# wubinzzu/NeuRec

Measured on NVIDIA H100. Metric: triplets/sec, higher is better.
Workload: dtype f32

## Files before the change

### neurec_b200/csrc/epoch.cuh

```cuda
#pragma once
#include "common.cuh"
#include "philox.cuh"

namespace nrc {

constexpr int kFeistelRounds = 8;

struct Feistel {
    uint32_t key[kFeistelRounds];
    uint64_t n;
    int32_t bits_l;
    int32_t bits_r;
    int32_t shuffle;
};

__host__ __device__ __forceinline__ uint32_t feistel_mix(uint32_t r, uint32_t key) {
    const uint32_t v = r ^ key;
    const uint64_t prod = (uint64_t)0xD2511F53u * v;
    uint32_t f = (uint32_t)(prod >> 32) ^ (uint32_t)prod;
    f = (f ^ (f >> 15)) * 0x9E3779B1u;
    return f ^ (f >> 13);
}

__host__ __device__ __forceinline__ uint64_t feistel_once(const Feistel& F, uint64_t x) {
    int bl = F.bits_l, br = F.bits_r;
    uint32_t L = (uint32_t)(x >> br), R = (uint32_t)(x & ((1ull << br) - 1ull));
#pragma unroll
    for (int r = 0; r < kFeistelRounds; ++r) {
        const uint32_t nr = L ^ (feistel_mix(R, F.key[r]) & (uint32_t)((1ull << bl) - 1ull));
        L = R; R = nr;
        const int t = bl; bl = br; br = t;
    }
    return ((uint64_t)L << br) | R;
}

__host__ __device__ __forceinline__ int64_t feistel_perm(const Feistel& F, int64_t p) {
    if (!F.shuffle) return p;
    uint64_t x = (uint64_t)p;
    do { x = feistel_once(F, x); } while (x >= F.n);
    return (int64_t)x;
}

struct EpochSpec {
    const int64_t* tptr;
    const int32_t* tidx;
    const int32_t* users;
    const int32_t* pos;
    int64_t n_pos;
    int64_t n_samples;
    int32_t neg_num;
    int32_t num_items;
    int32_t pairwise;
    uint64_t seed, stream_id;
    Feistel perm;
};

__device__ __forceinline__ void epoch_sample(const EpochSpec& E, int64_t p, int k, int32_t& u, int32_t& item,
                                             int32_t& third) {
    const int64_t idx = feistel_perm(E.perm, p);
    if (E.pairwise) {
        u = __ldg(E.users + idx);
        item = __ldg(E.pos + idx);
        const int64_t beg = __ldg(E.tptr + u);
        third = philox_draw_excluding((uint64_t)(idx * E.neg_num + k), E.seed, E.stream_id, E.num_items,
                                      E.tidx + beg, __ldg(E.tptr + u + 1) - beg);
    } else if (idx < E.n_pos) {
        u = __ldg(E.users + idx);
        item = __ldg(E.pos + idx);
        third = __float_as_int(1.0f);
    } else {
        const int64_t t = idx - E.n_pos;
        const int64_t kk = t / E.n_pos, q = t - kk * E.n_pos;
        u = __ldg(E.users + q);
        const int64_t beg = __ldg(E.tptr + u);
        item = philox_draw_excluding((uint64_t)(q * E.neg_num + kk), E.seed, E.stream_id, E.num_items,
                                     E.tidx + beg, __ldg(E.tptr + u + 1) - beg);
        third = __float_as_int(0.0f);
    }
}

int feistel_init(Feistel& F, int64_t n, int shuffle, uint64_t seed, uint64_t epoch);
int epoch_spec_init(EpochSpec& E, const int64_t* tptr, const int32_t* tidx, const int32_t* users, const int32_t* pos,
                    int64_t n_pos, int32_t neg_num, int32_t num_items, int32_t pairwise, int32_t shuffle,
                    uint64_t seed, uint64_t stream_id);

__device__ __forceinline__ void grid_barrier(unsigned int* counter, unsigned int& target) {
    __syncthreads();
    if (threadIdx.x == 0) {
        target += gridDim.x;
        unsigned int seen;
        asm volatile("red.release.gpu.global.add.u32 [%0], 1;" ::"l"(counter) : "memory");
        do {
            asm volatile("ld.acquire.gpu.global.u32 %0, [%1];" : "=r"(seen) : "l"(counter) : "memory");
        } while (seen < target);
    }
    __syncthreads();
}

}
```

### neurec_b200/csrc/train_mf.cu

```cuda
#include <stdlib.h>

#include "common.cuh"
#include "epoch.cuh"
#include "learner.cuh"
#include "mf.cuh"
#include "optim.cuh"

namespace nrc {

template <bool PAIRWISE>
__global__ void __launch_bounds__(256)
mf_grad_kernel(const float* __restrict__ U, const float* __restrict__ V, int D, const int32_t* __restrict__ users,
               const int32_t* __restrict__ items, const int32_t* __restrict__ third, int64_t batch, int loss_kind,
               float reg, float* __restrict__ gU, float* __restrict__ gV, int32_t* __restrict__ tU,
               int32_t* __restrict__ tV, int32_t stamp, float* __restrict__ loss) {
    const int lane = threadIdx.x & 31;
    const int wib = threadIdx.x >> 5;
    const int wpb = blockDim.x >> 5;
    const float inv_b = 1.0f / (float)batch;
    float loss_acc = 0.0f;
    for (int64_t b = (int64_t)blockIdx.x * wpb + wib; b < batch; b += (int64_t)gridDim.x * wpb)
        loss_acc += mf_sample_grad<PAIRWISE, 0, false>(U, V, gU, gV, tU, tV, D, reg, loss_kind, lane, users[b], items[b],
                                                       third[b], inv_b, stamp);
    if (lane == 0 && loss) atomicAdd(loss, loss_acc);
}

struct RowShards {
    float* base[8];
    int32_t rows_per_shard;
    int32_t self;
    int32_t vec_remote;
    int32_t force_remote;
    float* hot;
    float* hot_delta;
    int32_t n_hot;
    template <bool SHARDED>
    __device__ __forceinline__ float* row(int32_t id, int D, bool& remote, float*& upd) const {
        if (id < n_hot) {
            remote = false;
            upd = hot_delta + (size_t)id * D;
            return hot + (size_t)id * D;
        }
        float* p = row<SHARDED>(id, D, remote);
        upd = p;
        return p;
    }
    template <bool SHARDED>
    __device__ __forceinline__ float* row(int32_t id, int D, bool& remote) const {
        if constexpr (!SHARDED) {
            remote = force_remote != 0;
            return base[0] + (size_t)id * D;
        } else {
            const int32_t owner = id / rows_per_shard;
            remote = owner != self || force_remote;
            float* b = base[0];
#pragma unroll
            for (int r = 1; r < 8; ++r) b = (owner == r) ? base[r] : b;
            return b + (size_t)(id - owner * rows_per_shard) * D;
        }
    }
};

template <int VEC>
__device__ __forceinline__ void red_row(float* p, const float (&d)[VEC], bool remote) {
    if (remote) {
#pragma unroll
        for (int t = 0; t < VEC; ++t) atomicAdd(p + t, d[t]);
        return;
    }
    red_vec<VEC>(p, d);
}

template <int VEC, bool SHARDED>
__global__ void __launch_bounds__(256)
mf_bpr_sgd_fused_kernel(const RowShards U, const RowShards V, const int32_t* __restrict__ users,
                        const int32_t* __restrict__ pos, const int32_t* __restrict__ neg, int64_t batch,
                        float lr, float reg, float* __restrict__ loss) {
    constexpr int D = 32 * VEC;
    const int lane = threadIdx.x & 31;
    const int64_t wpb = blockDim.x >> 5;
    float loss_acc = 0.0f;
    for (int64_t b = (int64_t)blockIdx.x * wpb + (threadIdx.x >> 5); b < batch; b += (int64_t)gridDim.x * wpb) {
        bool ru, ri, rj;
        float* pu = U.row<SHARDED>(users[b], D, ru) + lane * VEC;
        float* qi = V.row<SHARDED>(pos[b], D, ri) + lane * VEC;
        float* qj = V.row<SHARDED>(neg[b], D, rj) + lane * VEC;
        float a[VEC], bi[VEC], bj[VEC];
        ld_vec<VEC>(pu, a); ld_vec<VEC>(qi, bi); ld_vec<VEC>(qj, bj);
        float di = 0.f, dj = 0.f, sq = 0.f;
#pragma unroll
        for (int t = 0; t < VEC; ++t) {
            di = fmaf(a[t], bi[t], di);
            dj = fmaf(a[t], bj[t], dj);
            sq += a[t] * a[t] + bi[t] * bi[t] + bj[t] * bj[t];
        }
        di = warp_sum(di); dj = warp_sum(dj);
        const float x = di - dj;
        float l = neg_log_sigmoid(x);
        if (reg != 0.0f) l += reg * 0.5f * warp_sum(sq);
        loss_acc += l;
        const float g = neg_log_sigmoid_grad(x);
        float du[VEC], dvi[VEC], dvj[VEC];
#pragma unroll
        for (int t = 0; t < VEC; ++t) {
            du[t] = -lr * (g * (bi[t] - bj[t]) + reg * a[t]);
            dvi[t] = -lr * (g * a[t] + reg * bi[t]);
            dvj[t] = -lr * (-g * a[t] + reg * bj[t]);
        }
        red_row<VEC>(pu, du, ru && U.vec_remote == 0);
        red_row<VEC>(qi, dvi, ri && V.vec_remote == 0);
        red_row<VEC>(qj, dvj, rj && V.vec_remote == 0);
    }
    if (lane == 0 && loss) atomicAdd(loss, loss_acc);
}

static int peer_red_mode() {
    static int vec = -1;
    if (vec < 0) { const char* e = getenv("NRC_PEER_VEC_RED"); vec = e ? atoi(e) : 1; }
    return vec;
}

static int launch_bpr_sgd(const RowShards& SU, const RowShards& SV, int dim, const int32_t* users,
                          const int32_t* pos, const int32_t* neg, int64_t batch, float lr, float reg, float* loss,
                          cudaStream_t st) {
    int64_t blocks = (batch + 7) / 8;
    const int64_t cap = (int64_t)sm_count() * 8;
    if (blocks > cap) blocks = cap;
    const unsigned gb = (unsigned)blocks;
#define NRC_LAUNCH_SGD(VEC, SH) \
    mf_bpr_sgd_fused_kernel<VEC, SH><<<gb, 256, 0, st>>>(SU, SV, users, pos, neg, batch, lr, reg, loss)
    const bool sharded = SU.rows_per_shard != 0;
    if (dim == 128) { if (sharded) NRC_LAUNCH_SGD(4, true); else NRC_LAUNCH_SGD(4, false); }
    else if (dim == 64) { if (sharded) NRC_LAUNCH_SGD(2, true); else NRC_LAUNCH_SGD(2, false); }
    else { if (sharded) NRC_LAUNCH_SGD(1, true); else NRC_LAUNCH_SGD(1, false); }
#undef NRC_LAUNCH_SGD
    NRC_CUDA_CHECK(cudaGetLastError());
    return NRC_OK;
}


template <int VEC>
constexpr int kSgdTierRows = 8192 / (32 * VEC);
template <int VEC>
constexpr size_t kSgdTierBytes = (size_t)2 * kSgdTierRows<VEC> * 32 * VEC * sizeof(float);

template <int VEC, bool SHARDED>
__device__ __forceinline__ void load_item(const RowShards& V, int32_t id, int nt, const float* s_val, int lane,
                                          float (&v)[VEC]) {
    if (id < nt) {
        ld_vec<VEC>(s_val + id * (32 * VEC) + lane * VEC, v);
    } else {
        bool remote;
        float* upd;
        ld_vec<VEC>(V.row<SHARDED>(id, 32 * VEC, remote, upd) + lane * VEC, v);
    }
}

template <int VEC, bool SHARDED>
__device__ __forceinline__ void update_item(const RowShards& V, int32_t id, int nt, float* s_dlt, int lane,
                                            const float (&d)[VEC]) {
    if (id < nt) {
#pragma unroll
        for (int t = 0; t < VEC; ++t) atomicAdd(s_dlt + id * (32 * VEC) + t * 32 + lane, d[t]);
    } else {
        bool remote;
        float* upd;
        V.row<SHARDED>(id, 32 * VEC, remote, upd);
        red_row<VEC>(upd + lane * VEC, d, remote && V.vec_remote == 0);
    }
}

constexpr int kStreamThreads = 768;

template <int VEC, bool SHARDED>
__global__ void __launch_bounds__(kStreamThreads, 1)
mf_bpr_sgd_stream_kernel(float* __restrict__ U_local, const RowShards V, const EpochSpec E, int64_t first,
                         int64_t count, float lr, float reg, float* __restrict__ loss) {
    constexpr int D = 32 * VEC, CH = kStreamThreads, T = kSgdTierRows<VEC>;
    constexpr int TPW = 2;
    __shared__ int32_t s_u[CH], s_i[CH], s_j[CH];
    extern __shared__ __align__(16) float s_tier[];
    float* const s_val = s_tier;
    float* const s_dlt = s_tier + T * D;
    const int lane = threadIdx.x & 31, warp = threadIdx.x >> 5;
    const int nt = V.n_hot < T ? V.n_hot : T;
    for (int e = threadIdx.x; e < nt * D / 4; e += blockDim.x) {
        reinterpret_cast<float4*>(s_val)[e] = reinterpret_cast<const float4*>(V.hot)[e];
        reinterpret_cast<float4*>(s_dlt)[e] = make_float4(0.f, 0.f, 0.f, 0.f);
    }
    const int64_t lo = count * blockIdx.x / gridDim.x, hi = count * (blockIdx.x + 1) / gridDim.x;
    float loss_acc = 0.0f;
    for (int64_t c0 = lo; c0 < hi; c0 += CH) {
        const int n = (hi - c0 < CH) ? (int)(hi - c0) : CH;
        if ((int)threadIdx.x < n) {
            int32_t u, i, j;
            epoch_sample(E, first + c0 + threadIdx.x, 0, u, i, j);
            s_u[threadIdx.x] = u; s_i[threadIdx.x] = i; s_j[threadIdx.x] = j;
        }
        __syncthreads();
        for (int t0 = warp * TPW; t0 < n; t0 += (kStreamThreads / 32) * TPW) {
            float a[TPW][VEC], b[TPW][VEC], c[TPW][VEC];
#pragma unroll
            for (int k = 0; k < TPW; ++k) {
                const int t = (t0 + k < n) ? t0 + k : t0;
                ld_vec<VEC>(U_local + (size_t)s_u[t] * D + lane * VEC, a[k]);
                load_item<VEC, SHARDED>(V, s_i[t], nt, s_val, lane, b[k]);
                load_item<VEC, SHARDED>(V, s_j[t], nt, s_val, lane, c[k]);
            }
            float di[TPW], dj[TPW], sq[TPW];
#pragma unroll
            for (int k = 0; k < TPW; ++k) {
                di[k] = 0.f; dj[k] = 0.f; sq[k] = 0.f;
#pragma unroll
                for (int t = 0; t < VEC; ++t) {
                    di[k] = fmaf(a[k][t], b[k][t], di[k]); dj[k] = fmaf(a[k][t], c[k][t], dj[k]);
                    sq[k] += a[k][t] * a[k][t] + b[k][t] * b[k][t] + c[k][t] * c[k][t];
                }
                di[k] = warp_sum(di[k]); dj[k] = warp_sum(dj[k]);
            }
#pragma unroll
            for (int k = 0; k < TPW; ++k) {
                if (t0 + k >= n) break;
                const int t = t0 + k;
                const float x = di[k] - dj[k];
                float l = neg_log_sigmoid(x);
                if (reg != 0.0f) l += reg * 0.5f * warp_sum(sq[k]);
                loss_acc += l;
                const float g = neg_log_sigmoid_grad(x);
                float du[VEC], dvi[VEC], dvj[VEC];
#pragma unroll
                for (int q = 0; q < VEC; ++q) {
                    du[q] = -lr * (g * (b[k][q] - c[k][q]) + reg * a[k][q]);
                    dvi[q] = -lr * (g * a[k][q] + reg * b[k][q]);
                    dvj[q] = -lr * (-g * a[k][q] + reg * c[k][q]);
                }
                red_row<VEC>(U_local + (size_t)s_u[t] * D + lane * VEC, du, false);
                update_item<VEC, SHARDED>(V, s_i[t], nt, s_dlt, lane, dvi);
                update_item<VEC, SHARDED>(V, s_j[t], nt, s_dlt, lane, dvj);
            }
        }
        __syncthreads();
    }
    __syncthreads();
    for (int e = threadIdx.x; e < nt * 32; e += blockDim.x) {
        const int r = e >> 5, l = e & 31;
        float d[VEC];
        bool any = false;
#pragma unroll
        for (int t = 0; t < VEC; ++t) { d[t] = s_dlt[r * D + t * 32 + l]; any |= d[t] != 0.0f; }
        if (any) red_row<VEC>(V.hot_delta + (size_t)r * D + l * VEC, d, false);
    }
    if (lane == 0 && loss) atomicAdd(loss, loss_acc);
}

template <int VEC, bool SH>
static int launch_stream(float* U_local, const RowShards& SV, const EpochSpec& E, int64_t first, int64_t count, float lr,
                         float reg, float* loss, cudaStream_t st) {
    constexpr size_t smem = kSgdTierBytes<VEC>;
    static int64_t grid_cap = 0;
    if (!grid_cap) {
        NRC_CUDA_CHECK(cudaFuncSetAttribute(mf_bpr_sgd_stream_kernel<VEC, SH>, cudaFuncAttributeMaxDynamicSharedMemorySize,
                                            (int)smem));
        int per_sm = 0;
        NRC_CUDA_CHECK(cudaOccupancyMaxActiveBlocksPerMultiprocessor(&per_sm, mf_bpr_sgd_stream_kernel<VEC, SH>, kStreamThreads, smem));
        NRC_REQUIRE(per_sm > 0, NRC_E_CUDA, "mf_bpr_sgd_stream_kernel does not fit on an SM");
        grid_cap = (int64_t)per_sm * sm_count();
    }
    int64_t blocks = (count + kStreamThreads - 1) / kStreamThreads;
    if (blocks > grid_cap) blocks = grid_cap;
    mf_bpr_sgd_stream_kernel<VEC, SH><<<(unsigned)blocks, kStreamThreads, smem, st>>>(U_local, SV, E, first, count, lr, reg, loss);
    NRC_CUDA_CHECK(cudaGetLastError());
    return NRC_OK;
}

static int launch_bpr_sgd_stream(float* U_local, const RowShards& SV, int dim, const EpochSpec& E, int64_t first,
                                 int64_t count, float lr, float reg, float* loss, cudaStream_t st) {
    const bool sharded = SV.rows_per_shard != 0;
#define NRC_STREAM(VEC) (sharded ? launch_stream<VEC, true>(U_local, SV, E, first, count, lr, reg, loss, st) \
                                 : launch_stream<VEC, false>(U_local, SV, E, first, count, lr, reg, loss, st))
    if (dim == 128) return NRC_STREAM(4);
    if (dim == 64) return NRC_STREAM(2);
    return NRC_STREAM(1);
#undef NRC_STREAM
}

template <int VEC>
__device__ __forceinline__ void lazy_adam_row(float* var, float* m, float* v, const float (&x)[VEC], float (&mm)[VEC],
                                              float (&vv)[VEC], const float (&g)[VEC], float lr_t, float b1, float b2,
                                              float eps) {
    float out[VEC];
#pragma unroll
    for (int t = 0; t < VEC; ++t) {
        mm[t] = b1 * mm[t] + (1.0f - b1) * g[t];
        vv[t] = b2 * vv[t] + (1.0f - b2) * g[t] * g[t];
        out[t] = x[t] - lr_t * mm[t] / (sqrtf(vv[t]) + eps);
    }
    st_vec<VEC>(m, mm); st_vec<VEC>(v, vv); st_vec<VEC>(var, out);
}

template <int VEC>
__global__ void __launch_bounds__(256, 3)
mf_bpr_lazy_adam_stream_kernel(float* __restrict__ U, float* __restrict__ mU, float* __restrict__ vU, float* __restrict__ V,
                               float* __restrict__ mV, float* __restrict__ vV, const EpochSpec E, int64_t first, int64_t count,
                               float lr_t, float b1, float b2, float eps, float reg, float* __restrict__ loss) {
    constexpr int D = 32 * VEC;
    constexpr int CH = 256;
    __shared__ int32_t s_u[CH], s_i[CH], s_j[CH];
    const int lane = threadIdx.x & 31, warp = threadIdx.x >> 5;
    float loss_acc = 0.0f;
    for (int64_t c0 = (int64_t)blockIdx.x * CH; c0 < count; c0 += (int64_t)gridDim.x * CH) {
        const int n = (count - c0 < CH) ? (int)(count - c0) : CH;
        if ((int)threadIdx.x < n) {
            int32_t u, i, j;
            epoch_sample(E, first + c0 + threadIdx.x, 0, u, i, j);
            s_u[threadIdx.x] = u; s_i[threadIdx.x] = i; s_j[threadIdx.x] = j;
        }
        __syncthreads();
        for (int t = warp; t < n; t += 8) {
            const size_t ou = (size_t)s_u[t] * D + lane * VEC, oi = (size_t)s_i[t] * D + lane * VEC,
                         oj = (size_t)s_j[t] * D + lane * VEC;
            float a[VEC], bi[VEC], bj[VEC], mu[VEC], vu[VEC], mi[VEC], vi[VEC], mj[VEC], vj[VEC];
            ld_vec<VEC>(U + ou, a); ld_vec<VEC>(V + oi, bi); ld_vec<VEC>(V + oj, bj);
            ld_vec<VEC>(mU + ou, mu); ld_vec<VEC>(vU + ou, vu);
            ld_vec<VEC>(mV + oi, mi); ld_vec<VEC>(vV + oi, vi);
            ld_vec<VEC>(mV + oj, mj); ld_vec<VEC>(vV + oj, vj);
            float di = 0.f, dj = 0.f, sq = 0.f;
#pragma unroll
            for (int c = 0; c < VEC; ++c) {
                di = fmaf(a[c], bi[c], di); dj = fmaf(a[c], bj[c], dj);
                sq += a[c] * a[c] + bi[c] * bi[c] + bj[c] * bj[c];
            }
            di = warp_sum(di); dj = warp_sum(dj);
            const float x = di - dj;
            float l = neg_log_sigmoid(x);
            if (reg != 0.0f) l += reg * 0.5f * warp_sum(sq);
            loss_acc += l;
            const float g = neg_log_sigmoid_grad(x);
            float gu[VEC], gi[VEC], gj[VEC];
#pragma unroll
            for (int c = 0; c < VEC; ++c) {
                gu[c] = g * (bi[c] - bj[c]) + reg * a[c];
                gi[c] = g * a[c] + reg * bi[c];
                gj[c] = -g * a[c] + reg * bj[c];
            }
            lazy_adam_row<VEC>(U + ou, mU + ou, vU + ou, a, mu, vu, gu, lr_t, b1, b2, eps);
            lazy_adam_row<VEC>(V + oi, mV + oi, vV + oi, bi, mi, vi, gi, lr_t, b1, b2, eps);
            lazy_adam_row<VEC>(V + oj, mV + oj, vV + oj, bj, mj, vj, gj, lr_t, b1, b2, eps);
        }
        __syncthreads();
    }
    if (lane == 0 && loss) atomicAdd(loss, loss_acc);
}

static int grad_grid(int64_t batch) {
    const int wpb = 8;
    int64_t blocks = (batch + wpb - 1) / wpb;
    const int64_t cap = (int64_t)sm_count() * 8;
    if (blocks > cap) blocks = cap;
    if (blocks < 1) blocks = 1;
    return (int)blocks;
}

}

using namespace nrc;

extern "C" int nrc_mf_pairwise_grad(const float* user_table, const float* item_table, int32_t dim,
                                    const int32_t* users, const int32_t* pos_items,
                                    const int32_t* neg_items, int64_t batch, int32_t loss_kind,
                                    float reg, float* grad_user, float* grad_item,
                                    int32_t* touched_user, int32_t* touched_item, int32_t stamp,
                                    float* loss, void* stream) {
    NRC_REQUIRE(loss_kind == NRC_LOSS_BPR || loss_kind == NRC_LOSS_HINGE ||
                    loss_kind == NRC_LOSS_SQUARE,
                NRC_E_VALUE, "please choose a suitable loss function");
    NRC_REQUIRE(dim > 0 && batch >= 0, NRC_E_VALUE, "dim must be positive, batch >= 0");
    if (batch == 0) return NRC_OK;
    mf_grad_kernel<true><<<grad_grid(batch), 256, 0, as_stream(stream)>>>(
        user_table, item_table, dim, users, pos_items, neg_items, batch, loss_kind, reg, grad_user,
        grad_item, touched_user, touched_item, stamp, loss);
    NRC_CUDA_CHECK(cudaGetLastError());
    return NRC_OK;
}

extern "C" int nrc_mf_pointwise_grad(const float* user_table, const float* item_table, int32_t dim,
                                     const int32_t* users, const int32_t* items,
                                     const float* labels, int64_t batch, int32_t loss_kind,
                                     float reg, float* grad_user, float* grad_item,
                                     int32_t* touched_user, int32_t* touched_item, int32_t stamp,
                                     float* loss, void* stream) {
    NRC_REQUIRE(loss_kind == NRC_LOSS_CROSS_ENTROPY || loss_kind == NRC_LOSS_SQUARE, NRC_E_VALUE,
                "please choose a suitable loss function");
    NRC_REQUIRE(dim > 0 && batch >= 0, NRC_E_VALUE, "dim must be positive, batch >= 0");
    if (batch == 0) return NRC_OK;
    mf_grad_kernel<false><<<grad_grid(batch), 256, 0, as_stream(stream)>>>(
        user_table, item_table, dim, users, items, reinterpret_cast<const int32_t*>(labels), batch, loss_kind, reg,
        grad_user, grad_item, touched_user, touched_item, stamp, loss);
    NRC_CUDA_CHECK(cudaGetLastError());
    return NRC_OK;
}

extern "C" int nrc_mf_bpr_sgd_fused(float* user_table, float* item_table, int32_t dim,
                                    const int32_t* users, const int32_t* pos_items,
                                    const int32_t* neg_items, int64_t batch, float lr, float reg,
                                    float* loss, void* stream) {
    NRC_REQUIRE(dim == 32 || dim == 64 || dim == 128, NRC_E_LIMIT,
                "the fused single-pass step supports dim 32, 64 or 128 (got %d)", dim);
    NRC_REQUIRE(batch >= 0, NRC_E_VALUE, "batch must be >= 0");
    if (batch == 0) return NRC_OK;
    RowShards SU{}, SV{};
    SU.base[0] = user_table; SV.base[0] = item_table;
    return launch_bpr_sgd(SU, SV, dim, users, pos_items, neg_items, batch, lr, reg, loss, as_stream(stream));
}

extern "C" int nrc_mf_bpr_sgd_sharded(float* const* user_shards, float* const* item_shards, int32_t world,
                                      int32_t self_rank, int64_t users_per_shard, int64_t items_per_shard, int32_t dim,
                                      const int32_t* users, const int32_t* pos_items, const int32_t* neg_items,
                                      int64_t batch, float lr, float reg, float* loss, void* stream) {
    NRC_REQUIRE(world >= 1 && world <= 8, NRC_E_LIMIT, "world %d outside [1, 8]", world);
    NRC_REQUIRE(self_rank >= 0 && self_rank < world, NRC_E_VALUE, "self_rank %d outside [0, %d)", self_rank, world);
    NRC_REQUIRE(user_shards != nullptr && item_shards != nullptr, NRC_E_VALUE, "shard pointer arrays are NULL");
    NRC_REQUIRE(users_per_shard > 0 && items_per_shard > 0 && users_per_shard < (1ll << 31) &&
                    items_per_shard < (1ll << 31) && users_per_shard * world < (1ll << 31) &&
                    items_per_shard * world < (1ll << 31),
                NRC_E_LIMIT, "global row ids must fit int32");
    NRC_REQUIRE(dim == 32 || dim == 64 || dim == 128, NRC_E_LIMIT, "fused SGD supports dim 32, 64, 128 (got %d)", dim);
    if (batch <= 0) return NRC_OK;
    RowShards SU{}, SV{};
    for (int r = 0; r < world; ++r) {
        NRC_REQUIRE(user_shards[r] != nullptr && item_shards[r] != nullptr, NRC_E_VALUE, "shard %d is NULL", r);
        SU.base[r] = user_shards[r];
        SV.base[r] = item_shards[r];
    }
    SU.rows_per_shard = (int32_t)users_per_shard;
    SV.rows_per_shard = (int32_t)items_per_shard;
    SU.self = SV.self = self_rank;
    SU.vec_remote = SV.vec_remote = peer_red_mode();
    return launch_bpr_sgd(SU, SV, dim, users, pos_items, neg_items, batch, lr, reg, loss, as_stream(stream));
}

extern "C" int nrc_mf_bpr_sgd_epoch_hot(float* user_table, float* const* item_shards, int32_t world, int32_t self_rank,
                                    int64_t items_per_shard, int32_t dim, const int64_t* train_indptr,
                                    const int32_t* train_indices, const int32_t* pos_users, const int32_t* pos_items,
                                    int64_t n_pos, int32_t num_items, int32_t shuffle, uint64_t seed, uint64_t epoch,
                                    int64_t first, int64_t count, float lr, float reg, float* loss, float* hot, float* hot_delta,
                                    int32_t n_hot, void* stream) {
    NRC_REQUIRE(world >= 1 && world <= 8, NRC_E_LIMIT, "world %d outside [1, 8]", world);
    NRC_REQUIRE(self_rank >= 0 && self_rank < world, NRC_E_VALUE, "self_rank %d outside [0, %d)", self_rank, world);
    NRC_REQUIRE(user_table != nullptr && item_shards != nullptr, NRC_E_VALUE, "table pointers are NULL");
    NRC_REQUIRE(dim == 32 || dim == 64 || dim == 128, NRC_E_LIMIT, "fused SGD supports dim 32, 64, 128 (got %d)", dim);
    NRC_REQUIRE(world == 1 || (items_per_shard > 0 && items_per_shard * world < (1ll << 31) &&
                               items_per_shard * world >= num_items),
                NRC_E_VALUE, "items_per_shard %lld x world %d must cover num_items %d and fit int32",
                (long long)items_per_shard, world, num_items);
    EpochSpec E;
    int rc = epoch_spec_init(E, train_indptr, train_indices, pos_users, pos_items, n_pos, 1, num_items, 1, shuffle, seed,
                             epoch);
    if (rc) return rc;
    NRC_REQUIRE(first >= 0 && count >= 0 && first + count <= n_pos, NRC_E_VALUE,
                "[first, first + count) = [%lld, %lld) outside the epoch's %lld triplets", (long long)first,
                (long long)(first + count), (long long)n_pos);
    if (count == 0) return NRC_OK;
    RowShards SV{};
    for (int r = 0; r < world; ++r) {
        NRC_REQUIRE(item_shards[r] != nullptr, NRC_E_VALUE, "item shard %d is NULL", r);
        SV.base[r] = item_shards[r];
    }
    SV.rows_per_shard = world > 1 ? (int32_t)items_per_shard : 0;
    SV.self = self_rank;
    NRC_REQUIRE(n_hot >= 0 && n_hot <= num_items && (n_hot == 0 || (hot != nullptr && hot_delta != nullptr)), NRC_E_VALUE,
                "n_hot %d needs 0 <= n_hot <= num_items and the replica / delta buffers", n_hot);
    SV.hot = hot; SV.hot_delta = hot_delta; SV.n_hot = n_hot;
    {
        static int vec = -1, force = -1;
        if (vec < 0) vec = peer_red_mode();
        if (force < 0) { const char* e = getenv("NRC_FORCE_REMOTE_PATH"); force = e ? atoi(e) : 0; }
        SV.vec_remote = vec;
        SV.force_remote = force;
    }
    return launch_bpr_sgd_stream(user_table, SV, dim, E, first, count, lr, reg, loss, as_stream(stream));
}

extern "C" int nrc_mf_bpr_sgd_epoch(float* user_table, float* const* item_shards, int32_t world, int32_t self_rank,
                                    int64_t items_per_shard, int32_t dim, const int64_t* train_indptr,
                                    const int32_t* train_indices, const int32_t* pos_users, const int32_t* pos_items,
                                    int64_t n_pos, int32_t num_items, int32_t shuffle, uint64_t seed, uint64_t epoch,
                                    int64_t first, int64_t count, float lr, float reg, float* loss, void* stream) {
    return nrc_mf_bpr_sgd_epoch_hot(user_table, item_shards, world, self_rank, items_per_shard, dim, train_indptr,
                                    train_indices, pos_users, pos_items, n_pos, num_items, shuffle, seed, epoch, first,
                                    count, lr, reg, loss, nullptr, nullptr, 0, stream);
}

namespace nrc {
__global__ void __launch_bounds__(256) hot_apply_kernel(float4* __restrict__ hot, float4* __restrict__ delta, int64_t n4) {
    for (int64_t e = (int64_t)blockIdx.x * blockDim.x + threadIdx.x; e < n4; e += (int64_t)gridDim.x * blockDim.x) {
        float4 h = hot[e];
        const float4 d = delta[e];
        h.x += d.x; h.y += d.y; h.z += d.z; h.w += d.w;
        hot[e] = h;
        delta[e] = make_float4(0.f, 0.f, 0.f, 0.f);
    }
}
}

extern "C" int nrc_mf_hot_apply(float* hot, float* hot_delta, int64_t n_floats, void* stream) {
    NRC_REQUIRE(n_floats >= 0 && (n_floats & 3) == 0, NRC_E_VALUE, "n_floats %lld must be a multiple of 4", (long long)n_floats);
    if (n_floats == 0) return NRC_OK;
    NRC_REQUIRE(hot && hot_delta, NRC_E_VALUE, "replica / delta pointers are NULL");
    int64_t blocks = (n_floats / 4 + 255) / 256;
    const int64_t cap = (int64_t)sm_count() * 8;
    if (blocks > cap) blocks = cap;
    hot_apply_kernel<<<(unsigned)blocks, 256, 0, as_stream(stream)>>>(reinterpret_cast<float4*>(hot),
                                                                      reinterpret_cast<float4*>(hot_delta), n_floats / 4);
    NRC_CUDA_CHECK(cudaGetLastError());
    return NRC_OK;
}

extern "C" int nrc_mf_bpr_lazy_adam_epoch(float* user_table, float* user_m, float* user_v, float* item_table, float* item_m,
                                          float* item_v, int32_t dim, const int64_t* train_indptr,
                                          const int32_t* train_indices, const int32_t* pos_users, const int32_t* pos_items,
                                          int64_t n_pos, int32_t num_items, int32_t shuffle, uint64_t seed, uint64_t epoch,
                                          int64_t first, int64_t count, float lr_t, float beta1, float beta2, float eps,
                                          float reg, float* loss, void* stream) {
    NRC_REQUIRE(dim == 32 || dim == 64 || dim == 128, NRC_E_LIMIT, "lazy Adam supports dim 32, 64, 128 (got %d)", dim);
    NRC_REQUIRE(user_table && user_m && user_v && item_table && item_m && item_v, NRC_E_VALUE, "table / slot pointers are NULL");
    EpochSpec E;
    int rc = epoch_spec_init(E, train_indptr, train_indices, pos_users, pos_items, n_pos, 1, num_items, 1, shuffle, seed,
                             epoch);
    if (rc) return rc;
    NRC_REQUIRE(first >= 0 && count >= 0 && first + count <= n_pos, NRC_E_VALUE,
                "[first, first + count) = [%lld, %lld) outside the epoch's %lld triplets", (long long)first,
                (long long)(first + count), (long long)n_pos);
    if (count == 0) return NRC_OK;
    int64_t blocks = (count + 255) / 256;
    const int64_t cap = (int64_t)sm_count() * 8;
    if (blocks > cap) blocks = cap;
    cudaStream_t st = as_stream(stream);
#define NRC_LAZY(VEC) mf_bpr_lazy_adam_stream_kernel<VEC><<<(unsigned)blocks, 256, 0, st>>>( \
        user_table, user_m, user_v, item_table, item_m, item_v, E, first, count, lr_t, beta1, beta2, eps, reg, loss)
    if (dim == 128) NRC_LAZY(4); else if (dim == 64) NRC_LAZY(2); else NRC_LAZY(1);
#undef NRC_LAZY
    NRC_CUDA_CHECK(cudaGetLastError());
    return NRC_OK;
}

extern "C" int nrc_enable_peer_access(int32_t peer_device) {
    int cur = 0;
    NRC_CUDA_CHECK(cudaGetDevice(&cur));
    if (cur == peer_device) return NRC_OK;
    int can = 0;
    NRC_CUDA_CHECK(cudaDeviceCanAccessPeer(&can, cur, peer_device));
    NRC_REQUIRE(can, NRC_E_CUDA, "device %d cannot access device %d", cur, peer_device);
    const cudaError_t e = cudaDeviceEnablePeerAccess(peer_device, 0);
    if (e == cudaErrorPeerAccessAlreadyEnabled) { cudaGetLastError(); return NRC_OK; }
    NRC_CUDA_CHECK(e);
    return NRC_OK;
}

extern "C" int nrc_opt_apply_rows(int32_t opt_kind, float* var, float* grad, float* slot0,
                                  float* slot1, const int32_t* touched, int32_t stamp, int64_t rows,
                                  int32_t dim, const float* hyper_host, void* stream) {
    OptLaunch L;
    int rc = opt_launch_init(L, opt_kind, hyper_host);
    if (rc) return rc;
    rc = opt_launch_add(L, var, grad, slot0, slot1, touched, rows, dim, 0);
    if (rc) return rc;
    return opt_launch_run(L, stamp, as_stream(stream));
}

extern "C" int nrc_opt_apply_multi(int32_t opt_kind, int32_t n_vars, float* const* var,
                                   float* const* grad, float* const* slot0, float* const* slot1,
                                   const int32_t* const* touched, const int64_t* rows,
                                   const int32_t* dims, const int32_t* dense_var, int32_t stamp,
                                   const float* hyper_host, void* stream) {
    OptLaunch L;
    int rc = opt_launch_init(L, opt_kind, hyper_host);
    if (rc) return rc;
    for (int i = 0; i < n_vars; ++i) {
        rc = opt_launch_add(L, var[i], grad[i], slot0 ? slot0[i] : nullptr,
                            slot1 ? slot1[i] : nullptr, touched ? touched[i] : nullptr, rows[i],
                            dims[i], dense_var ? dense_var[i] : 0);
        if (rc) return rc;
    }
    return opt_launch_run(L, stamp, as_stream(stream));
}

extern "C" int nrc_mf_train_epoch(float* user_table, float* item_table, int32_t num_users,
                                  int32_t num_items, int32_t dim, const int32_t* users,
                                  const int32_t* items, const void* third, int64_t n,
                                  int32_t batch_size, int32_t pairwise, int32_t loss_kind, float reg,
                                  int32_t opt_kind, const float* lr_t_host, const float* hyper_host,
                                  float* grad_user, float* grad_item, int32_t* touched_user,
                                  int32_t* touched_item, float* slot0_user, float* slot1_user,
                                  float* slot0_item, float* slot1_item, int32_t first_stamp,
                                  float* step_loss, void* stream) {
    NRC_REQUIRE(batch_size > 0, NRC_E_VALUE, "batch_size should be a positive integeral value");
    NRC_REQUIRE(n >= 0 && dim > 0, NRC_E_VALUE, "n >= 0 and dim > 0 required");
    cudaStream_t st = as_stream(stream);
    const int64_t steps = (n + batch_size - 1) / batch_size;
    if (steps == 0) return NRC_OK;
    NRC_CUDA_CHECK(cudaMemsetAsync(step_loss, 0, (size_t)steps * sizeof(float), st));
    float hyper[4] = {hyper_host[0], hyper_host[1], hyper_host[2], hyper_host[3]};
    for (int64_t s = 0; s < steps; ++s) {
        const int64_t off = s * batch_size;
        const int64_t bs = (n - off < batch_size) ? (n - off) : batch_size;
        const int32_t stamp = first_stamp + (int32_t)s;
        int rc;
        if (pairwise)
            rc = nrc_mf_pairwise_grad(user_table, item_table, dim, users + off, items + off,
                                      reinterpret_cast<const int32_t*>(third) + off, bs, loss_kind,
                                      reg, grad_user, grad_item, touched_user, touched_item, stamp,
                                      step_loss + s, stream);
        else
            rc = nrc_mf_pointwise_grad(user_table, item_table, dim, users + off, items + off,
                                       reinterpret_cast<const float*>(third) + off, bs, loss_kind,
                                       reg, grad_user, grad_item, touched_user, touched_item, stamp,
                                       step_loss + s, stream);
        if (rc) return rc;
        if (opt_kind == NRC_OPT_ADAM) hyper[0] = lr_t_host[s];
        OptLaunch L;
        rc = opt_launch_init(L, opt_kind, hyper);
        if (rc) return rc;
        opt_launch_add(L, user_table, grad_user, slot0_user, slot1_user, touched_user, num_users, dim, 0);
        opt_launch_add(L, item_table, grad_item, slot0_item, slot1_item, touched_item, num_items, dim, 0);
        rc = opt_launch_run(L, stamp, st);
        if (rc) return rc;
    }
    return NRC_OK;
}

extern "C" int nrc_mf_train_step_host(float* user_table, float* item_table, int32_t num_users,
                                      int32_t num_items, int32_t dim, const int32_t* users_host,
                                      const int32_t* items_host, const void* third_host,
                                      int64_t batch, int32_t pairwise, int32_t loss_kind, float reg,
                                      int32_t opt_kind, const float* hyper_host, float* grad_user,
                                      float* grad_item, int32_t* touched_user,
                                      int32_t* touched_item, float* slot0_user, float* slot1_user,
                                      float* slot0_item, float* slot1_item, int32_t stamp,
                                      void* staging, float* loss_host, void* stream) {
    NRC_REQUIRE(batch > 0 && dim > 0, NRC_E_VALUE, "batch and dim must be positive");
    cudaStream_t st = as_stream(stream);
    int32_t* d_users = reinterpret_cast<int32_t*>(staging);
    int32_t* d_items = d_users + batch;
    int32_t* d_third = d_items + batch;
    float* d_loss = reinterpret_cast<float*>(d_third + batch);
    const size_t nb = (size_t)batch * sizeof(int32_t);
    NRC_CUDA_CHECK(cudaMemcpyAsync(d_users, users_host, nb, cudaMemcpyHostToDevice, st));
    NRC_CUDA_CHECK(cudaMemcpyAsync(d_items, items_host, nb, cudaMemcpyHostToDevice, st));
    NRC_CUDA_CHECK(cudaMemcpyAsync(d_third, third_host, nb, cudaMemcpyHostToDevice, st));
    NRC_CUDA_CHECK(cudaMemsetAsync(d_loss, 0, sizeof(float), st));
    int rc;
    if (pairwise)
        rc = nrc_mf_pairwise_grad(user_table, item_table, dim, d_users, d_items, d_third, batch,
                                  loss_kind, reg, grad_user, grad_item, touched_user, touched_item,
                                  stamp, d_loss, stream);
    else
        rc = nrc_mf_pointwise_grad(user_table, item_table, dim, d_users, d_items,
                                   reinterpret_cast<const float*>(d_third), batch, loss_kind, reg,
                                   grad_user, grad_item, touched_user, touched_item, stamp, d_loss,
                                   stream);
    if (rc) return rc;
    OptLaunch L;
    rc = opt_launch_init(L, opt_kind, hyper_host);
    if (rc) return rc;
    opt_launch_add(L, user_table, grad_user, slot0_user, slot1_user, touched_user, num_users, dim, 0);
    opt_launch_add(L, item_table, grad_item, slot0_item, slot1_item, touched_item, num_items, dim, 0);
    rc = opt_launch_run(L, stamp, st);
    if (rc) return rc;
    NRC_CUDA_CHECK(cudaMemcpyAsync(loss_host, d_loss, sizeof(float), cudaMemcpyDeviceToHost, st));
    NRC_CUDA_CHECK(cudaStreamSynchronize(st));
    return NRC_OK;
}
```

### profiles/step_rows.py

```python
import argparse
import json
import os
import sys

import numpy as np

ROOT = os.path.dirname(os.path.dirname(os.path.abspath(__file__)))
sys.path.insert(0, ROOT)


def main():
    import bench
    import oracle
    ap = argparse.ArgumentParser()
    ap.add_argument("--step", type=int, default=0)
    args = ap.parse_args()
    cfg = bench.ShardedCfg
    ptr, idx = bench.synth_shard_csr(cfg, 0, 1, device="cpu")
    users = np.repeat(np.arange(len(ptr) - 1, dtype=np.int32), np.diff(ptr))
    wu, wi, wj = oracle.epoch_build(ptr, idx, users, idx, 1, cfg.items_per_gpu, True, True, bench.SEED, 0)
    lo = args.step * cfg.batch
    u, i, j = wu[lo:lo + cfg.batch], wi[lo:lo + cfg.batch], wj[lo:lo + cfg.batch, 0]
    n_hot = bench.n_hot_of(cfg, 1)
    cu = np.bincount(u, minlength=cfg.users_per_gpu)
    items = np.concatenate([i, j])
    ci = np.bincount(items[items >= n_hot], minlength=cfg.items_per_gpu)
    once_u = int((cu[u] == 1).sum())
    cold_i, cold_j = i[i >= n_hot], j[j >= n_hot]
    once_i, once_j = int((ci[cold_i] == 1).sum()), int((ci[cold_j] == 1).sum())
    total = len(u) + len(cold_i) + len(cold_j)
    print(json.dumps({
        "step": args.step, "triplets": len(u), "n_hot": n_hot,
        "user_updates": len(u), "user_touched_once": once_u / len(u),
        "negative_updates_outside_head": len(cold_j), "negatives_in_head": float((j < n_hot).mean()),
        "negative_touched_once": once_j / len(cold_j),
        "positive_updates_outside_head": len(cold_i), "positive_touched_once": once_i / len(cold_i),
        "positives_in_head": int((i < n_hot).sum()), "positives_in_shared_memory_tier": int((i < 64).sum()),
        "in_place_updates": total, "touched_once": once_u + once_i + once_j,
        "touched_once_share": (once_u + once_i + once_j) / total}))


if __name__ == "__main__":
    main()
```

Measured before the change: 837.9 million.

## Replace atomic user-row updates with plain stores for users touched once per chunk

For each sampled triplet, the sampler inverts the Feistel shuffle over the user's other interactions to check whether any fall in the same launch range. Users with short rows that appear only once get flagged, and their row update becomes a plain add and vector store instead of an atomic reduction. This aims to cut global atomic traffic on the user table, but adds up to 32 inverse-Feistel evaluations per sample during sampling. Flagged users' rows are read and then overwritten non-atomically, which stays correct only if the once-per-range check holds. The diff also extends a profiling script to report this rule's coverage.

```diff
diff --git a/neurec_b200/csrc/epoch.cuh b/neurec_b200/csrc/epoch.cuh
--- a/neurec_b200/csrc/epoch.cuh
+++ b/neurec_b200/csrc/epoch.cuh
@@ -38,6 +38,26 @@
     if (!F.shuffle) return p;
     uint64_t x = (uint64_t)p;
     do { x = feistel_once(F, x); } while (x >= F.n);
+    return (int64_t)x;
+}
+
+static_assert(kFeistelRounds % 2 == 0, "feistel_once_inv assumes the halves end at their initial widths");
+__host__ __device__ __forceinline__ uint64_t feistel_once_inv(const Feistel& F, uint64_t x) {
+    int bl = F.bits_l, br = F.bits_r;
+    uint32_t L = (uint32_t)(x >> br), R = (uint32_t)(x & ((1ull << br) - 1ull));
+#pragma unroll
+    for (int r = kFeistelRounds - 1; r >= 0; --r) {
+        const uint32_t pl = R ^ (feistel_mix(L, F.key[r]) & (uint32_t)((1ull << br) - 1ull));
+        R = L; L = pl;
+        const int t = bl; bl = br; br = t;
+    }
+    return ((uint64_t)L << br) | R;
+}
+
+__host__ __device__ __forceinline__ int64_t feistel_perm_inv(const Feistel& F, int64_t q) {
+    if (!F.shuffle) return q;
+    uint64_t x = (uint64_t)q;
+    do { x = feistel_once_inv(F, x); } while (x >= F.n);
     return (int64_t)x;
 }
 
diff --git a/neurec_b200/csrc/train_mf.cu b/neurec_b200/csrc/train_mf.cu
--- a/neurec_b200/csrc/train_mf.cu
+++ b/neurec_b200/csrc/train_mf.cu
@@ -170,12 +170,40 @@
     }
 }
 
+__device__ __forceinline__ float add_as_red(float x, float d) {
+    float r;
+    asm("add.rn.ftz.f32 %0, %1, %2;" : "=f"(r) : "f"(x), "f"(d));
+    return r;
+}
+
+constexpr int64_t kOnceMaxRow = 32;
+constexpr int32_t kUserOnce = INT32_MIN;
+
+__device__ __forceinline__ void stream_sample(const EpochSpec& E, int64_t p, int64_t first, int64_t count, bool user_once,
+                                              int32_t& u, int32_t& item, int32_t& third) {
+    const int64_t idx = feistel_perm(E.perm, p);
+    u = __ldg(E.users + idx);
+    item = __ldg(E.pos + idx);
+    const int64_t beg = __ldg(E.tptr + u), end = __ldg(E.tptr + u + 1);
+    third = philox_draw_excluding((uint64_t)(idx * E.neg_num), E.seed, E.stream_id, E.num_items, E.tidx + beg, end - beg);
+    if (user_once && end - beg <= kOnceMaxRow) {
+        bool alone = true;
+#pragma unroll 1
+        for (int64_t q = beg; q < end; ++q) {
+            if (q == idx) continue;
+            const int64_t r = feistel_perm_inv(E.perm, q);
+            alone &= (uint64_t)(r - first) >= (uint64_t)count;
+        }
+        if (alone) u |= kUserOnce;
+    }
+}
+
 constexpr int kStreamThreads = 768;
 
 template <int VEC, bool SHARDED>
 __global__ void __launch_bounds__(kStreamThreads, 1)
 mf_bpr_sgd_stream_kernel(float* __restrict__ U_local, const RowShards V, const EpochSpec E, int64_t first,
-                         int64_t count, float lr, float reg, float* __restrict__ loss) {
+                         int64_t count, int user_once, float lr, float reg, float* __restrict__ loss) {
     constexpr int D = 32 * VEC, CH = kStreamThreads, T = kSgdTierRows<VEC>;
     constexpr int TPW = 2;
     __shared__ int32_t s_u[CH], s_i[CH], s_j[CH];
@@ -194,7 +222,7 @@
         const int n = (hi - c0 < CH) ? (int)(hi - c0) : CH;
         if ((int)threadIdx.x < n) {
             int32_t u, i, j;
-            epoch_sample(E, first + c0 + threadIdx.x, 0, u, i, j);
+            stream_sample(E, first + c0 + threadIdx.x, first, count, user_once != 0, u, i, j);
             s_u[threadIdx.x] = u; s_i[threadIdx.x] = i; s_j[threadIdx.x] = j;
         }
         __syncthreads();
@@ -203,7 +231,7 @@
 #pragma unroll
             for (int k = 0; k < TPW; ++k) {
                 const int t = (t0 + k < n) ? t0 + k : t0;
-                ld_vec<VEC>(U_local + (size_t)s_u[t] * D + lane * VEC, a[k]);
+                ld_vec<VEC>(U_local + (size_t)(s_u[t] & ~kUserOnce) * D + lane * VEC, a[k]);
                 load_item<VEC, SHARDED>(V, s_i[t], nt, s_val, lane, b[k]);
                 load_item<VEC, SHARDED>(V, s_j[t], nt, s_val, lane, c[k]);
             }
@@ -234,7 +262,15 @@
                     dvi[q] = -lr * (g * a[k][q] + reg * b[k][q]);
                     dvj[q] = -lr * (-g * a[k][q] + reg * c[k][q]);
                 }
-                red_row<VEC>(U_local + (size_t)s_u[t] * D + lane * VEC, du, false);
+                const int32_t su = s_u[t];
+                float* const pu = U_local + (size_t)(su & ~kUserOnce) * D + lane * VEC;
+                if (su & kUserOnce) {
+#pragma unroll
+                    for (int q = 0; q < VEC; ++q) du[q] = add_as_red(a[k][q], du[q]);
+                    st_vec<VEC>(pu, du);
+                } else {
+                    red_row<VEC>(pu, du, false);
+                }
                 update_item<VEC, SHARDED>(V, s_i[t], nt, s_dlt, lane, dvi);
                 update_item<VEC, SHARDED>(V, s_j[t], nt, s_dlt, lane, dvj);
             }
@@ -254,8 +290,8 @@
 }
 
 template <int VEC, bool SH>
-static int launch_stream(float* U_local, const RowShards& SV, const EpochSpec& E, int64_t first, int64_t count, float lr,
-                         float reg, float* loss, cudaStream_t st) {
+static int launch_stream(float* U_local, const RowShards& SV, const EpochSpec& E, int64_t first, int64_t count,
+                         int user_once, float lr, float reg, float* loss, cudaStream_t st) {
     constexpr size_t smem = kSgdTierBytes<VEC>;
     static int64_t grid_cap = 0;
     if (!grid_cap) {
@@ -268,7 +304,8 @@
     }
     int64_t blocks = (count + kStreamThreads - 1) / kStreamThreads;
     if (blocks > grid_cap) blocks = grid_cap;
-    mf_bpr_sgd_stream_kernel<VEC, SH><<<(unsigned)blocks, kStreamThreads, smem, st>>>(U_local, SV, E, first, count, lr, reg, loss);
+    mf_bpr_sgd_stream_kernel<VEC, SH><<<(unsigned)blocks, kStreamThreads, smem, st>>>(U_local, SV, E, first, count,
+                                                                                      user_once, lr, reg, loss);
     NRC_CUDA_CHECK(cudaGetLastError());
     return NRC_OK;
 }
@@ -276,8 +313,9 @@
 static int launch_bpr_sgd_stream(float* U_local, const RowShards& SV, int dim, const EpochSpec& E, int64_t first,
                                  int64_t count, float lr, float reg, float* loss, cudaStream_t st) {
     const bool sharded = SV.rows_per_shard != 0;
-#define NRC_STREAM(VEC) (sharded ? launch_stream<VEC, true>(U_local, SV, E, first, count, lr, reg, loss, st) \
-                                 : launch_stream<VEC, false>(U_local, SV, E, first, count, lr, reg, loss, st))
+    const int user_once = E.pos == E.tidx ? 1 : 0;
+#define NRC_STREAM(VEC) (sharded ? launch_stream<VEC, true>(U_local, SV, E, first, count, user_once, lr, reg, loss, st) \
+                                 : launch_stream<VEC, false>(U_local, SV, E, first, count, user_once, lr, reg, loss, st))
     if (dim == 128) return NRC_STREAM(4);
     if (dim == 64) return NRC_STREAM(2);
     return NRC_STREAM(1);
diff --git a/profiles/step_rows.py b/profiles/step_rows.py
--- a/profiles/step_rows.py
+++ b/profiles/step_rows.py
@@ -26,12 +26,21 @@
     items = np.concatenate([i, j])
     ci = np.bincount(items[items >= n_hot], minlength=cfg.items_per_gpu)
     once_u = int((cu[u] == 1).sum())
+    n = len(idx)
+    inv = np.empty(n, np.int64)
+    inv[oracle.shuffle_perm(n, bench.SEED, 0, True)] = np.arange(n)
+    visited = ((inv - lo) >= 0) & ((inv - lo) < cfg.batch)
+    per_row = np.add.reduceat(visited.astype(np.int64), ptr[:-1])
+    rule_u = int(((per_row[u] == 1) & (np.diff(ptr)[u] <= 32)).sum())
     cold_i, cold_j = i[i >= n_hot], j[j >= n_hot]
     once_i, once_j = int((ci[cold_i] == 1).sum()), int((ci[cold_j] == 1).sum())
     total = len(u) + len(cold_i) + len(cold_j)
+    bands = [0, 64, 256, 1024, 4096, n_hot]
+    head = {"%d-%d" % (a, b): int(((items >= a) & (items < b)).sum()) for a, b in zip(bands[:-1], bands[1:]) if b > a}
     print(json.dumps({
         "step": args.step, "triplets": len(u), "n_hot": n_hot,
         "user_updates": len(u), "user_touched_once": once_u / len(u),
+        "user_touched_once_kernel_rule": rule_u / len(u), "head_accesses_by_rank": head,
         "negative_updates_outside_head": len(cold_j), "negatives_in_head": float((j < n_hot).mean()),
         "negative_touched_once": once_j / len(cold_j),
         "positive_updates_outside_head": len(cold_i), "positive_touched_once": once_i / len(cold_i),
```

Result: faster. 865.6 million, median of 6 (+3.3%).
